# Justin900429/autonomous_driving_with_diffusion_model

Measured on AMD Instinct MI355X. Metric: denoising-steps/sec, higher is better.
Workload: dtype f32

## Files before the change

autonomous_driving_with_diffusion_model_amd/csrc/conv2d_hs.hip:

```cpp
#include <type_traits>
#include <stdlib.h>

#include "adx_common.h"
#include "conv2d_internal.h"
#include "conv2d_hs_common.h"

namespace adx {

template <bool AFFINE = true>
__device__ __forceinline__ void cells_store32(float (&v)[16], const float* sc, const float* sh, int cl0, const float (*res8)[8],
                                              bool relu, __amdgpu_buffer_rsrc_t yrsrc, uint32_t vcell, uint32_t so, uint32_t cplane,
                                              float& amax) {
  float lm = 0.f;
#pragma unroll
  for (int i = 0; i < 2; ++i)
#pragma unroll
    for (int j = 0; j < 4; ++j) {
      const auto sw = __builtin_amdgcn_permlane32_swap(f2u(v[8 * i + j]), f2u(v[8 * i + 4 + j]), false, false);
      v[8 * i + j] = u2f(sw[0]);
      v[8 * i + 4 + j] = u2f(sw[1]);
    }
#pragma unroll
  for (int i = 0; i < 2; ++i) {
    float o[8];
// ... 325 lines not shown
        if (a.relu) v = v > 0.f ? v : 0.f;
        lm = fp16_amax(lm, v);
        __builtin_amdgcn_raw_buffer_store_b32(__builtin_bit_cast(uint32_t, v), yrsrc, voff[rr], cbase_o + cu * plane_ob, 0);
        if (DS) {
          const float d = (adm[rr][half][r] + adl[rr][half][r] * (1.f / kLoScale)) * xs_inv;
          const float dv = d * ss[2 * kHsCout + cl] + ss[3 * kHsCout + cl];
          lm = fp16_amax(lm, dv);
          __builtin_amdgcn_raw_buffer_store_b32(__builtin_bit_cast(uint32_t, dv), drsrc, voff[rr], cbase_o + cu * plane_ob, 0);
        }
      }
    amax = fp16_amax(amax, voff[rr] != kOut ? lm : 0.f);
  }
  range_flag(a.status, out_of_fp16(amax));
}

#ifdef ADX_HS_TRACE
__device__ unsigned long long g_hs_trace[8 * 16384];
__device__ __forceinline__ void hs_trace(int slot) {
  if (threadIdx.x == 0 && blockIdx.x < 16384) g_hs_trace[blockIdx.x * 8 + slot] = __builtin_readcyclecounter();
}
__device__ __forceinline__ void hs_trace_id() {
  if (threadIdx.x == 0 && blockIdx.x < 16384) {
    unsigned hw, xcc;
    asm volatile("s_getreg_b32 %0, hwreg(HW_REG_HW_ID)" : "=s"(hw));
    asm volatile("s_getreg_b32 %0, hwreg(HW_REG_XCC_ID)" : "=s"(xcc));
    g_hs_trace[blockIdx.x * 8 + 7] = ((unsigned long long)xcc << 32) | hw;
  }
}
#define HS_TRACE(slot) hs_trace(slot)
#else
#define HS_TRACE(slot)
#endif

template <int MODE, int STATS = 0, bool XCELLS = false, bool YCELLS = false, bool VR = false, bool PAIR = false>
__global__ void __launch_bounds__(MODE == 0 ? 256 : 512, 2) conv2d_hs3x3_kernel(const Conv2dArgs a) {
  static_assert(!PAIR || (MODE == 0 && STATS == 0), "the PAIR form is the plain 4-wave tile");
  constexpr bool VROW = YCELLS || VR;
  constexpr int NT = MODE == 0 ? 256 : 512;
  constexpr int TH = MODE == 1 ? 16 : 8;
  constexpr int CT = MODE == 2 ? 2 : 1;
  constexpr int K = 3, PH = TH + 2, PW = 34, PLANE = PH * PW, NITEM = 2 * PLANE;
  constexpr int PIT = (NITEM + NT - 1) / NT;
  constexpr int NW = 9 * 256, WST = PAIR ? 2 * 256 : 3 * 256 * CT;
  constexpr int WIT = (WST + NT - 1) / NT;
  static_assert(PIT <= K, "a patch slice travels with each stage of a chunk");
  extern __shared__ __attribute__((aligned(16))) unsigned char smem_raw[];
  u32x4* patch = reinterpret_cast<u32x4*>(smem_raw);
  u32x4* wl = patch + 2 * 4 * PLANE;
  float* ss = reinterpret_cast<float*>(wl + 2 * WST);
  u32x4* dummy = reinterpret_cast<u32x4*>(ss + 2 * 64 * CT + 8);
  float* bsl = reinterpret_cast<float*>(dummy + 3);
  const int tid = threadIdx.x, lane = tid & 63;
  const int wave = __builtin_amdgcn_readfirstlane(tid >> 6);
  const int rowpair = MODE == 2 ? (wave & 3) : wave, slab = MODE == 2 ? (wave >> 2) : 0;
#ifdef ADX_HS_TRACE
  hs_trace_id();
#endif
  HS_TRACE(0);
  int bid = blockIdx.x;
  {
    const int per = gridDim.x >> 3;
    if (bid < per * 8) bid = (bid & 7) * per + (bid >> 3);
  }
  int kpart = 0;
  if (a.ksplit > 1) { kpart = bid % a.ksplit; bid /= a.ksplit; }
  const int ct = bid % a.cout_tiles; bid /= a.cout_tiles;
  const int tx = bid % a.tiles_x; bid /= a.tiles_x;
  const int ty = bid % a.tiles_y; bid /= a.tiles_y;
  const int n = VROW ? 0 : bid;
  const int oy0 = ty * TH, ox0 = tx * kTileW;
  const int iy0 = oy0 - a.pad, ix0 = ox0 - a.pad;
  const int cout0 = (ct * CT + slab) * kHsCout;
  const int l31 = lane & 31, khalf = lane >> 5;
  const int vx0 = tx * kTileW;
  const int ecol = PAIR ? 16 * ((lane >> 4) & 1) + (lane & 15) : l31;
  const int vl = vx0 + ecol;
  auto vdiv = [&](int v) { return (int)(((float)v + 0.5f) * a.inv_vw); };
  const int nl = VROW ? vdiv(vl) : 0, xl = VROW ? vl - nl * a.vw : 0;
  const bool lane_valid = !VROW || (nl < a.N && xl < a.W);
  const size_t hw = (size_t)a.H * a.W;
  const int nchunks_all = a.cin_pad / kHsCC;
  const int nchunks = a.ksplit > 1 ? a.cper : nchunks_all;
  const int chunk0 = kpart * nchunks;
  const float* xin = a.x + ((size_t)n * a.Cin + (size_t)chunk0 * kHsCC) * hw;
  const int nstages = nchunks * K;
  const u32x4* wsrc = reinterpret_cast<const u32x4*>(a.w) + ((size_t)ct * CT * nchunks_all + chunk0) * NW;
  constexpr uint32_t kOutside = 0xC0000000u;
  const __amdgpu_buffer_rsrc_t xrsrc = __builtin_amdgcn_make_buffer_rsrc(
      const_cast<float*>(xin), 0,
      (int)(uint32_t)((VROW ? (size_t)a.N * a.Cin : (size_t)(a.Cin - chunk0 * kHsCC)) * hw * sizeof(float)), 0x00020000);
  const uint32_t plane_bytes = (uint32_t)(hw * sizeof(float));
  uint32_t goff[PIT];
  int pcell[PIT];
#pragma unroll
  for (int k = 0; k < PIT; ++k) {
    const int e = tid + NT * k;
    const int hg = e >= PLANE ? 1 : 0;
    const int p = e - hg * PLANE;
    const int py = p / PW, px = p - py * PW;
    const int iy = iy0 + py;
    int ix = ix0 + px, ni = n;
    if constexpr (VROW) {
      const int v = vx0 - 1 + px;
      ni = vdiv(v < 0 ? 0 : v);
      ix = v - ni * a.vw;
    }
    const bool ok = e < NITEM && iy >= 0 && iy < a.H && ix >= 0 && ix < a.W && ni < a.N;
    const size_t ioff = VROW ? (size_t)ni * a.Cin * hw * sizeof(float) : 0;
    goff[k] = !ok ? kOutside
                  : XCELLS ? (uint32_t)(ioff + hg * 8 * hw * sizeof(float) + ((size_t)iy * a.W + ix) * 16)
                           : (uint32_t)(ioff + (hg * 8 * hw + (size_t)iy * a.W + ix) * sizeof(float));
    pcell[k] = e < NITEM ? hg * 2 * PLANE + p : -1;
  }
  int wsrc_off[WIT], wdst[WIT];
#pragma unroll
  for (int k = 0; k < WIT; ++k) {
    const int e = tid + NT * k;
    const int sl = e / 768, within = e - sl * 768;
    const bool ok = e < WST;
    wsrc_off[k] = ok ? sl * nchunks_all * NW + within : 0;
    wdst[k] = ok ? e : -1;
  }
  float ssv = 0.f;
  if (tid < 2 * 64 * CT) {
    const int half = tid / (64 * CT), cc = tid - half * 64 * CT;
    const int c = ct * CT * kHsCout + cc;
    ssv = a.scale == nullptr ? (half == 0 ? 1.f : 0.f) : (half == 0 ? a.scale[c] : a.shift[c]);
  }
  float bsv = 0.f;
  if (STATS == 2 && tid < 4 * 64 * CT) {
    const int which = tid / (64 * CT), cc = tid - which * 64 * CT;
    const int c = ct * CT * kHsCout + cc;
    const float mu = a.bs_mean[c], rs = a.bs_rstd[c];
    const float sc = a.bs_gamma[c] * rs;
    bsv = which == 0 ? mu : (which == 1 ? rs : (which == 2 ? sc : __builtin_fmaf(-mu, sc, a.bs_beta[c])));
  }
  float xs = 1.f, xs_inv = 1.f;
  if (a.x_amax != nullptr && a.x_amax_n < 0) {
    xs_inv = reinterpret_cast<const float*>(a.x_amax)[1];
  } else if (a.x_amax != nullptr) {
    uint32_t* red = reinterpret_cast<uint32_t*>(ss + 2 * 64 * CT);
    uint32_t b = 0;
    for (int i = tid; i < a.x_amax_n; i += NT) b = a.x_amax[i] > b ? a.x_amax[i] : b;
#pragma unroll
    for (int off = 32; off > 0; off >>= 1) {
// ... 38 lines not shown
#pragma unroll
    for (int k = 0; k < WIT; ++k) {
      u32x4* d = (WST % NT == 0 || wdst[k] >= 0) ? wl + buf * WST + wdst[k] : dummy + 2;
      *d = wv[set][k];
    }
  };
  auto load_p = [&](int chunk, int k, int set) {
    const uint32_t cbase = (uint32_t)chunk * kHsCC * plane_bytes;
    if (XCELLS) {
      const u32x4 h4 = __builtin_amdgcn_raw_buffer_load_b128(xrsrc, goff[k], cbase, 0);
      const u32x4 l4 = __builtin_amdgcn_raw_buffer_load_b128(xrsrc, goff[k], cbase + 4 * plane_bytes, 0);
#pragma unroll
      for (int j = 0; j < 4; ++j) {
        pv[set][j] = u2f(h4[j]);
        pv[set][4 + j] = u2f(l4[j]);
      }
    } else {
#pragma unroll
      for (int j = 0; j < 8; ++j)
        pv[set][j] = __builtin_bit_cast(float, __builtin_amdgcn_raw_buffer_load_b32(xrsrc, goff[k], cbase + j * plane_bytes, 0));
    }
  };
  auto store_p = [&](int set, int k, int buf) {
    u32x4 hi, lo;
    if (XCELLS) {
#pragma unroll
      for (int j = 0; j < 4; ++j) {
        hi[j] = __builtin_bit_cast(uint32_t, pv[set][j]);
        lo[j] = __builtin_bit_cast(uint32_t, pv[set][4 + j]);
      }
    } else {
      split8(pv[set], xs, hi, lo);
    }
    u32x4* pd = patch + buf * 4 * PLANE + pcell[k];
    u32x4* d0 = pcell[k] >= 0 ? pd : dummy;
    u32x4* d1 = pcell[k] >= 0 ? pd + PLANE : dummy + 1;
    *d0 = hi;
    *d1 = lo;
  };

  auto half4 = [](uint32_t h0, uint32_t h1, uint32_t l0, uint32_t l1, float* out) {
    const float inv = 1.f / kLoScale;
    asm("v_fma_mix_f32 %0, %1, %2, %3 op_sel:[0,0,0] op_sel_hi:[1,0,1]" : "=v"(out[0]) : "v"(l0), "s"(inv), "v"(h0));
    asm("v_fma_mix_f32 %0, %1, %2, %3 op_sel:[1,0,1] op_sel_hi:[1,0,1]" : "=v"(out[1]) : "v"(l0), "s"(inv), "v"(h0));
    asm("v_fma_mix_f32 %0, %1, %2, %3 op_sel:[0,0,0] op_sel_hi:[1,0,1]" : "=v"(out[2]) : "v"(l1), "s"(inv), "v"(h1));
    asm("v_fma_mix_f32 %0, %1, %2, %3 op_sel:[1,0,1] op_sel_hi:[1,0,1]" : "=v"(out[3]) : "v"(l1), "s"(inv), "v"(h1));
  };

  const int pb_lane = khalf * 2 * PLANE + (rowpair * 2) * PW + l31;
  const int wa_lane = slab * 768 + khalf * 64 + l31;

  load_w(0, 0);
  store_w(0, 0);
#pragma unroll
  for (int k = 0; k < PIT; ++k) { load_p(0, k, 0); store_p(0, k, 0); }
  load_w(1, 1);
  if (tid < 2 * 64 * CT) ss[tid] = ssv;
  if (STATS == 2 && tid < 4 * 64 * CT) bsl[tid] = bsv;
  load_p(1, 0, 1);
  HS_TRACE(1);
  __syncthreads();
  HS_TRACE(2);

  if constexpr (PAIR) {
    const int j = lane & 15, kq = lane >> 4, ts = kq >> 1, kh2 = kq & 1;
    const int npairs = nchunks >> 1;
    f32x4 am[4][4], al[4][4];
#pragma unroll
    for (int cb = 0; cb < 4; ++cb)
#pragma unroll
      for (int pb = 0; pb < 4; ++pb)
#pragma unroll
        for (int i = 0; i < 4; ++i) { am[cb][pb][i] = 0.f; al[cb][pb][i] = 0.f; }
    const u32x4* pb_g[3];
#pragma unroll
    for (int g = 0; g < 3; ++g) {
      const HsPairTap t0 = hs_pair_stage(3 * g).tap[0], t1 = hs_pair_stage(3 * g).tap[1];
      pb_g[g] = patch + kh2 * 2 * PLANE + (rowpair * 2) * PW + j + (ts ? t1.odd * 4 * PLANE + t1.kh * PW : t0.odd * 4 * PLANE + t0.kh * PW);
    }
    const int wa_pair = ts * 256 + kh2 * 64 + j;
    auto load_runs = [&](int o0, int o1, int set) {
      wv[set][0] = wsrc[o0 + tid];
      wv[set][1] = wsrc[o1 + tid];
    };
    auto pair_stages = [&](const int par, const int pair) __attribute__((always_inline)) {
      const bool more = pair + 1 < npairs;
#pragma unroll
      for (int i = 0; i < 9; ++i) {
        const int gp = (i + par) & 1;
        const HsPairStage st = hs_pair_stage(i), nx = hs_pair_stage((i + 1) % 9);
        if (i + 2 < 9) load_runs(hs_pair_run(pair, i + 2, 0), hs_pair_run(pair, i + 2, 1), gp);
        else load_runs(more ? hs_pair_run(pair + 1, i + 2 - 9, 0) : hs_pair_run(pair, 8, 0), more ? hs_pair_run(pair + 1, i + 2 - 9, 1) : hs_pair_run(pair, 8, 1), gp);
        if (nx.pround >= 0) {
          const int c = 2 * pair + 1 + (i == 8 ? 2 : nx.pnext);
          load_p(c < nchunks ? c : nchunks - 1, nx.pround, gp);
        }
        __builtin_amdgcn_sched_barrier(0);
        const u32x4* pb0 = pb_g[i / 3] + i % 3;
        const u32x4* wa0 = wl + gp * WST + wa_pair;
        f16x8 A[2][4], B[2][4];
#pragma unroll
        for (int pl = 0; pl < 2; ++pl) {
#pragma unroll
          for (int cb = 0; cb < 4; ++cb) A[pl][cb] = __builtin_bit_cast(f16x8, wa0[pl * 128 + cb * 16]);
#pragma unroll
          for (int pb = 0; pb < (XCELLS ? 4 : 2); ++pb) B[pl][pb] = __builtin_bit_cast(f16x8, pb0[pl * PLANE + (pb >> 1) * PW + (pb & 1) * 16]);
        }
#pragma unroll
        for (int pb = 0; pb < 4; ++pb) {
          if (!XCELLS && pb == 1) {
            __builtin_amdgcn_sched_barrier(0);
// ... 17 lines not shown
        __syncthreads();
      }
    };
    int pair = 0;
    for (; pair + 1 < npairs; pair += 2) {
      pair_stages(0, pair);
      pair_stages(1, pair + 1);
    }
    if (pair < npairs) pair_stages(0, pair);

    const int ox = VROW ? xl : ox0 + ecol;
    const uint32_t plane_ob = (uint32_t)(a.OH * a.OW) * (uint32_t)sizeof(float);
    const uint32_t cplane = (uint32_t)(a.OH * a.OW) * 16u;
    const size_t img = (size_t)n * a.Cout * a.OH * a.OW;
    const int img_bytes = (int)(uint32_t)((VROW ? (uint32_t)a.N : 1u) * (uint32_t)a.Cout * plane_ob);
    const uint32_t img_off = VROW ? (uint32_t)nl * (uint32_t)a.Cout * plane_ob : 0u;
    const __amdgpu_buffer_rsrc_t yrsrc = __builtin_amdgcn_make_buffer_rsrc(a.y + img, 0, img_bytes, 0x00020000);
    const __amdgpu_buffer_rsrc_t rrsrc = __builtin_amdgcn_make_buffer_rsrc(
        const_cast<float*>(a.res != nullptr ? a.res + img : a.y), 0, a.res != nullptr ? img_bytes : 0, 0x00020000);
    const uint32_t cbase_o = (uint32_t)cout0 * plane_ob;
    const uint32_t cell0 = (uint32_t)(cout0 >> 3) * 2u * cplane;
    const bool rcells = YCELLS && a.res_cells;
    bool inside[2];
    uint32_t vout[2], vres[2];
#pragma unroll
    for (int rr = 0; rr < 2; ++rr) {
      const int oy = oy0 + rowpair * 2 + rr;
      inside[rr] = lane_valid && oy < a.OH && ox < a.OW;
      const uint32_t pix = (uint32_t)(oy * a.OW + ox);
      const uint32_t vc = img_off + pix * 16u + (uint32_t)ts * 2u * cplane, vf = img_off + pix * 4u + (uint32_t)(8 * ts) * plane_ob;
      vout[rr] = !inside[rr] ? kOutside : (YCELLS ? vc : vf);
      vres[rr] = !inside[rr] ? kOutside : (rcells ? vc : vf);
    }
    uint32_t rraw[4][2][8];
#pragma unroll
    for (int cb = 0; cb < 4; ++cb)
#pragma unroll
      for (int rr = 0; rr < 2; ++rr) {
        if (rcells) {
          const uint32_t so = cell0 + (uint32_t)(2 * cb) * 2u * cplane;
          const u32x4 h4 = __builtin_amdgcn_raw_buffer_load_b128(rrsrc, vres[rr], so, 0);
          const u32x4 l4 = __builtin_amdgcn_raw_buffer_load_b128(rrsrc, vres[rr], so + cplane, 0);
#pragma unroll
          for (int c = 0; c < 4; ++c) { rraw[cb][rr][c] = h4[c]; rraw[cb][rr][4 + c] = l4[c]; }
        } else {
#pragma unroll
          for (int c = 0; c < 8; ++c)
            rraw[cb][rr][c] = __builtin_amdgcn_raw_buffer_load_b32(rrsrc, vres[rr], cbase_o + (uint32_t)(16 * cb + c) * plane_ob, 0);
        }
      }
    float amax = 0.f;
#pragma unroll
    for (int cb = 0; cb < 4; ++cb)
#pragma unroll
      for (int rr = 0; rr < 2; ++rr) {
        float o[8], r8[8];
#pragma unroll
        for (int i = 0; i < 4; ++i) {
          const int cl = 16 * cb + 4 * kq + i;
          float x = (am[cb][2 * rr][i] + al[cb][2 * rr][i] * (1.f / kLoScale)) * xs_inv;
          float y = (am[cb][2 * rr + 1][i] + al[cb][2 * rr + 1][i] * (1.f / kLoScale)) * xs_inv;
          x = x * ss[cl] + ss[64 + cl];
          y = y * ss[cl] + ss[64 + cl];
          const auto sw = __builtin_amdgcn_permlane16_swap(f2u(x), f2u(y), false, false);
          o[i] = u2f(sw[0]);
          o[4 + i] = u2f(sw[1]);
        }
        if (rcells) {
          half4(rraw[cb][rr][0], rraw[cb][rr][1], rraw[cb][rr][4], rraw[cb][rr][5], r8);
          half4(rraw[cb][rr][2], rraw[cb][rr][3], rraw[cb][rr][6], rraw[cb][rr][7], r8 + 4);
        } else {
#pragma unroll
          for (int c = 0; c < 8; ++c) r8[c] = u2f(rraw[cb][rr][c]);
        }
        float lm = 0.f;
#pragma unroll
        for (int c = 0; c < 8; ++c) {
          const float t = o[c] + r8[c];
          o[c] = a.relu ? __builtin_fmaxf(t, 0.f) : t;
          lm = fp16_amax(lm, o[c]);
        }
        amax = fp16_amax(amax, inside[rr] ? lm : 0.f);
        if constexpr (YCELLS) {
          u32x4 hi, lo;
          split8(o, 1.f, hi, lo);
          const uint32_t so = cell0 + (uint32_t)(2 * cb) * 2u * cplane;
          __builtin_amdgcn_raw_buffer_store_b128(hi, yrsrc, vout[rr], so, 0);
          __builtin_amdgcn_raw_buffer_store_b128(lo, yrsrc, vout[rr], so + cplane, 0);
          asm volatile("s_nop 0" ::"v"(hi), "v"(lo));
        } else {
#pragma unroll
          for (int c = 0; c < 8; ++c)
            __builtin_amdgcn_raw_buffer_store_b32(f2u(o[c]), yrsrc, vout[rr], cbase_o + (uint32_t)(16 * cb + c) * plane_ob, 0);
        }
      }
    range_flag(a.status, out_of_fp16(amax));
    return;
  }

  for (int cp = 0; cp < nchunks; cp += 2) {
#pragma unroll
    for (int i = 0; i < 6; ++i) {
      const int s = 3 * cp + i;
      const int kh = i % 3, cpar = (i / 3) & 1;
      const u32x4* pb0 = patch + cpar * 4 * PLANE + pb_lane;
      const u32x4* wa0 = wl + (i & 1) * WST + wa_lane;
      load_w(s + 2 < nstages ? s + 2 : nstages - 1, i & 1);
      if ((i + 1) % 3 < PIT) load_p(s + 4 < nstages ? (s + 4) / 3 : nchunks - 1, (i + 1) % 3, i & 1);
      __builtin_amdgcn_sched_barrier(0);
#pragma unroll
      for (int kw = 0; kw < K; ++kw) {
        f16x8 A[2][2], B[2][2];
#pragma unroll
        for (int pl = 0; pl < 2; ++pl) {
#pragma unroll
          for (int m = 0; m < 2; ++m) A[pl][m] = __builtin_bit_cast(f16x8, wa0[(kw * 2 + pl) * 128 + m * 32]);
#pragma unroll
          for (int r = 0; r < 2; ++r) B[pl][r] = __builtin_bit_cast(f16x8, pb0[pl * PLANE + (r + kh) * PW + kw]);
        }
#pragma unroll
        for (int r = 0; r < 2; ++r)
#pragma unroll
          for (int m = 0; m < 2; ++m) {
            accm[r][m] = hs_mfma(A[0][m], B[0][r], accm[r][m]);
            accl[r][m] = hs_mfma(A[0][m], B[1][r], accl[r][m]);
            accl[r][m] = hs_mfma(A[1][m], B[0][r], accl[r][m]);
          }
        if (kw == 0) {
          store_w((i + 1) & 1, (i + 1) & 1);
          if (i % 3 < PIT) store_p((i + 1) & 1, i % 3, ((i + 3) / 3) & 1);
        }
      }
      __syncthreads();
    }
  }

  HS_TRACE(3);
  const int ox = VROW ? xl : ox0 + ecol;
// ... 886 lines not shown

__global__ void __launch_bounds__(256) conv2d_split_reduce_kernel(const float* __restrict__ part, size_t part_stride, int nparts,
                                                                  const float* __restrict__ scale, const float* __restrict__ shift,
                                                                  const float* __restrict__ res, float* __restrict__ y,
                                                                  int cout, int plane4, size_t total4, int relu, uint32_t* status) {
  const size_t i = (size_t)blockIdx.x * 256 + threadIdx.x;
  if (i >= total4) return;
  const int c = (int)((i / plane4) % cout);
  f32x4 v = reinterpret_cast<const f32x4*>(part)[i];
  for (int p0 = 1; p0 < nparts; p0 += 8) {
    f32x4 t[8];
#pragma unroll
    for (int j = 0; j < 8; ++j) t[j] = reinterpret_cast<const f32x4*>(part + (size_t)(p0 + j < nparts ? p0 + j : 0) * part_stride)[i];
#pragma unroll
    for (int j = 0; j < 8; ++j)
      if (p0 + j < nparts) v += t[j];
  }
  const float sc = scale != nullptr ? scale[c] : 1.f, sh = shift != nullptr ? shift[c] : 0.f;
  v = v * sc + sh;
  if (res != nullptr) v += reinterpret_cast<const f32x4*>(res)[i];
  if (relu) {
#pragma unroll
    for (int k = 0; k < 4; ++k) v[k] = __builtin_fmaxf(v[k], 0.f);
  }
  reinterpret_cast<f32x4*>(y)[i] = v;
  float amax = 0.f;
#pragma unroll
  for (int k = 0; k < 4; ++k) amax = fp16_amax(amax, v[k]);
  range_flag(status, out_of_fp16(amax));
}

static constexpr size_t hs3x3_lds(int mode, int stats, bool pair = false) {
  const int th = mode == 1 ? 16 : 8, ct = mode == 2 ? 2 : 1;
  return (size_t)2 * 64 * (th + 2) * 34 + (size_t)2 * (pair ? 2 : 3 * ct) * 256 * 16 + (2 * 64 * ct + 8) * sizeof(float) + 48 +
         (stats == 2 ? 4 * 64 * ct * sizeof(float) : 0);
}
static_assert(hs3x3_lds(0, 2) <= 80 * 1024 && hs3x3_lds(1, 2) <= 160 * 1024 && hs3x3_lds(2, 2) <= 160 * 1024, "LDS budget");
static_assert(hs3x3_lds(0, 0, true) <= 80 * 1024, "LDS budget: two workgroups of the PAIR form per CU");

Hs3x3Plan conv2d_hs3x3_plan(const ConvSpec& L, const Hs3x3Query& q, const DebugSwitches& sw) {
  Hs3x3Plan p;
  p.admitted = q.fmt == 0;
  if (!hs_eligible(L, sw) || !(L.k == 3 && L.stride == 1 && L.pad == 1) || (L.cin_pad / kHsCC) % 2 != 0) return p;
  const int N = q.N, OH = q.H, OW = q.W, nchunks = L.cin_pad / kHsCC;
  int mode = L.cin < 256 ? 0 : (OH > 8 ? 1 : (L.cout % 128 == 0 ? 2 : 0));
  const long grid0 = (long)N * ceil_div(OH, 8) * ceil_div(OW, kTileW) * (L.cout / kHsCout);
  if (grid0 <= 256) mode = 0;
  if (sw.hs_mode >= 0 && !(sw.hs_mode == 2 && L.cout % 128 != 0)) mode = sw.hs_mode == 1 || sw.hs_mode == 2 ? sw.hs_mode : 0;
  const int th = mode == 1 ? 16 : 8, ct = mode == 2 ? 2 : 1;
  const bool xc = (q.fmt & kFmtXCells) != 0, yc = (q.fmt & kFmtYCells) != 0, rc = (q.fmt & kFmtResCells) != 0 && q.has_res;
  const bool xscaled = q.x_scale == kXScalePre;
  const bool in_ok = (size_t)N * L.cin * q.H * q.W * sizeof(float) < 0xC0000000u;
  const bool bytes_ok = in_ok && (size_t)N * L.cout * OH * OW * sizeof(float) < 0xC0000000u;
  const bool vfits = (long)N * (OW + 1) < (1L << 21);
  const int vw = N > 1 ? OW + 1 : OW;
  const int vtiles_x = (int)(((long)N * vw - (N > 1 ? 1 : 0) + kTileW - 1) / kTileW);
  const bool vrow_ok = sw.conv_vrow && N > 1 && vfits && bytes_ok;
  const bool q_shape = sw.hs_mode < 0 && L.cout % 128 == 0 && L.cin_pad % 64 == 0;
  const bool q_fp32out = q_shape && xc && !yc && !rc && !q.affine && vfits && bytes_ok;
  const bool q_train = q_fp32out && sw.train_cells >= 3 && !q.has_res && q.x_scale == kXScaleNone && q.bst_mask == 0;
  const bool q_dgrad = q_fp32out && sw.train_cells >= 5 && xscaled && !q.relu && (q.bst_mask == 2 || (q.bst_mask == 1 && q.bst_bits));
  const bool q_plain = q_shape && xc && yc && (!q.has_res || rc) && q.x_scale == kXScaleNone;
  const int stats_tiles = q_train || q_dgrad ? ceil_div(OH, kQTH) * vtiles_x
                                             : ceil_div(OH, th) * (!yc && !rc && vrow_ok ? vtiles_x : N * ceil_div(OW, kTileW));
  p.stats_need = (size_t)stats_tiles * (L.cout * 2 + L.cout / 64);
  const bool stats = q.stats_floats > 0 && p.stats_need <= q.stats_floats;
  const bool split_shape = mode == 0 && grid0 <= 64 && nchunks >= 8;
// ... 184 lines not shown
```

autonomous_driving_with_diffusion_model_amd/csrc/conv2d_hs16.hip:

```cpp
#include "adx_common.h"
#include "conv2d_internal.h"
#include "conv2d_hs_common.h"

namespace adx {

namespace {

typedef __attribute__((address_space(3))) void lds_void;

__device__ __forceinline__ f32x4 mfma16(f16x8 a, f16x8 b, f32x4 c) { return __builtin_amdgcn_mfma_f32_16x16x32_f16(a, b, c, 0, 0, 0); }

__device__ __forceinline__ void half4(uint32_t h0, uint32_t h1, uint32_t l0, uint32_t l1, float* out) {
  const float inv = 1.f / kLoScale;
  asm("v_fma_mix_f32 %0, %1, %2, %3 op_sel:[0,0,0] op_sel_hi:[1,0,1]" : "=v"(out[0]) : "v"(l0), "s"(inv), "v"(h0));
  asm("v_fma_mix_f32 %0, %1, %2, %3 op_sel:[1,0,1] op_sel_hi:[1,0,1]" : "=v"(out[1]) : "v"(l0), "s"(inv), "v"(h0));
  asm("v_fma_mix_f32 %0, %1, %2, %3 op_sel:[0,0,0] op_sel_hi:[1,0,1]" : "=v"(out[2]) : "v"(l1), "s"(inv), "v"(h1));
  asm("v_fma_mix_f32 %0, %1, %2, %3 op_sel:[1,0,1] op_sel_hi:[1,0,1]" : "=v"(out[3]) : "v"(l1), "s"(inv), "v"(h1));
}

}

template <bool DMA, int TRAIN = 0>
__global__ void __launch_bounds__(kQNT, 2) conv2d_hs3x3q_kernel(const Conv2dArgs a) {
  constexpr bool S2 = TRAIN == 3;
  static_assert(!S2 || DMA, "the stride-2 block entry stages with LDS-DMA only");
  constexpr int NT = kQNT, PW = kQPW, PLANE = DMA ? kQPlaneD : kQPlane, PP = DMA ? kQPlaneD : kQPlaneP, PIT = kQPit, WST = kQWst;
  constexpr int NPAIRS = DMA ? kQPairsD : kQPairs;
  constexpr int GST = DMA ? PP : 2 * PP, PLST = DMA ? 4 * PP : PP;
  extern __shared__ __attribute__((aligned(16))) unsigned char smem_raw[];
  u32x4* patch = reinterpret_cast<u32x4*>(smem_raw);
  u32x4* wl = patch + 2 * 8 * PP;
  float* ss = reinterpret_cast<float*>(wl + 2 * WST);
  u32x4* dummy = reinterpret_cast<u32x4*>(ss + 256);
  float* bsl = reinterpret_cast<float*>(dummy + 2);
  uint32_t* gnext = reinterpret_cast<uint32_t*>(bsl + 512);
  uint32_t* gpl = gnext + PIT * NT;
  const int tid = threadIdx.x, lane = tid & 63;
  const int wave = __builtin_amdgcn_readfirstlane(tid >> 6);
  const int rowpair = wave & 3, slab = wave >> 2;
  const int j = lane & 15, kq = lane >> 4;
  const int Qs = a.q_slots;
  const HsQWalk wk = hs3x3q_walk((int)(blockIdx.x & 7), (int)(blockIdx.x >> 3), a.ntiles);
  const int u_end = wk.end;
  int u = wk.first;
  if (u >= u_end) return;
  HsQUnit un = hs3x3q_unit(u, a.cout_tiles);
  int sp = un.sp, ct = un.ct;
  int ty = sp / a.tiles_x, tx = sp - ty * a.tiles_x;
  int oy0 = ty * kQTH, vx0 = tx * 32;
  auto vdiv = [&](int v) { return (int)(((float)v + 0.5f) * a.inv_vw); };
  const size_t hw = (size_t)a.H * a.W;
  const int nch16 = a.cin_pad / 16, nch32 = a.cin_pad / 32, nstages = nch32 * 9;
  constexpr uint32_t kOutside = 0xC0000000u;
  const __amdgpu_buffer_rsrc_t xrsrc = __builtin_amdgcn_make_buffer_rsrc(
      const_cast<float*>(a.x), 0, (int)(uint32_t)((size_t)a.N * a.Cin * hw * sizeof(float)), 0x00020000);
  const uint32_t plane_bytes = (uint32_t)(hw * sizeof(float));
  auto goff_of = [&](int t_, int k, int oy0_, int vx0_) -> uint32_t {
    const int e = t_ + NT * k;
    const int g = e / PLANE, p = e - g * PLANE;
    const int py = p / PW, px = p - py * PW;
// ... 104 lines not shown
    } else {
      pvh[set] = __builtin_amdgcn_raw_buffer_load_b128(xrsrc, go, cbase, 0);
      pvl[set] = __builtin_amdgcn_raw_buffer_load_b128(xrsrc, go, cbase + 4 * plane_bytes, 0);
    }
  };
  auto load_p = [&](int chunk, int k, int set) { load_p_at(chunk, k, set, goff[k]); };
  auto store_p = [&](int set, int k, int buf) {
    if constexpr (!DMA) {
      u32x4* pd = patch + buf * 8 * PP + pcell[k];
      u32x4* d0 = (k < PIT - 1 || pcell[k] >= 0) ? pd : dummy;
      u32x4* d1 = (k < PIT - 1 || pcell[k] >= 0) ? pd + PP : dummy + 1;
      *d0 = pvh[set];
      *d1 = pvl[set];
    }
  };


  if constexpr (S2) load_w_tap(ct, 0, kTap[0], 0);
  else load_w(0, 0);
  store_w(0, 0);
#pragma unroll
  for (int k = 0; k < PIT; ++k) { load_p(0, k, 0); store_p(0, k, 0); }
  if constexpr (!DMA) load_w(1, 1);
  load_consts(ct);
  if constexpr (DMA) asm volatile("s_waitcnt vmcnt(0)" ::: "memory");
  __syncthreads();

  bool bad = false;
  for (;;) {
  int zero_ = 0;
  asm volatile("" : "+s"(zero_));
  const int tl = tid + zero_;
  if constexpr (DMA && !S2) {
#pragma unroll
    for (int k = 0; k < PIT; ++k) goff[k] = goff_of(tl, k, oy0, vx0);
#pragma unroll
    for (int k = 0; k < 2; ++k) {
      const int e = tl + NT * k;
      const int sl = e >> 9, half16 = (e >> 8) & 1, within = e & 255;
      wsrc_off[k] = (((ct * 2 + sl) * nch16 + half16) * 9) * 256 + within;
    }
  }
  const int j_l = tl & 15, kq_l = (tl & 63) >> 4;
  const int pb_lane = kq_l * GST + (rowpair * 2) * PW + j_l;
  const int wa_lane = slab * 512 + (kq_l >> 1) * 256 + (kq_l & 1) * 64 + j_l;
  const int u_next = u + Qs;
  const bool has_next = DMA && u_next < u_end;
  const HsQUnit un_next = hs3x3q_unit(u_next, a.cout_tiles);
  const int sp_next = un_next.sp;
  const int ct_next = has_next ? un_next.ct : ct;
  const int wct_next = (ct_next - ct) * (2 * 9 * 256) * nch16;
  const int nty = sp_next / a.tiles_x, ntx = sp_next - nty * a.tiles_x;
  const int n_oy0 = nty * kQTH, n_vx0 = ntx * 32;
  if constexpr (S2) {
#pragma unroll
    for (int k = 0; k < PIT; ++k) {
      const uint32_t g10 = goff_s2(tl, k, oy0, vx0, 1, 0);
      gpl[(0 * PIT + k) * NT + tid] = goff_s2(tl, k, oy0, vx0, 1, 1);
      gpl[(1 * PIT + k) * NT + tid] = g10;
      gpl[(2 * PIT + k) * NT + tid] = goff_s2(tl, k, oy0, vx0, 0, 1);
      gpl[(3 * PIT + k) * NT + tid] = goff_s2(tl, k, oy0, vx0, 0, 0);
      gnext[k * NT + tid] = has_next ? goff_s2(tl, k, n_oy0, n_vx0, 1, 0) : g10;
    }
  } else if constexpr (DMA) {
#pragma unroll
    for (int k = 0; k < PIT; ++k) gnext[k * NT + tid] = has_next ? goff_of(tl, k, n_oy0, n_vx0) : goff[k];
  }
#pragma unroll
  for (int cb = 0; cb < 4; ++cb)
#pragma unroll
    for (int pb = 0; pb < 4; ++pb)
#pragma unroll
      for (int i = 0; i < 4; ++i) { accm[cb][pb][i] = 0.f; accl[cb][pb][i] = 0.f; }

  auto s2_stage = [&](const u32x4* pb0, const u32x4* wa0) {
    __builtin_amdgcn_sched_barrier(0);
    f16x8 A[2][4], B[2][4];
#pragma unroll
    for (int pl = 0; pl < 2; ++pl) {
#pragma unroll
      for (int cb = 0; cb < 4; ++cb) A[pl][cb] = __builtin_bit_cast(f16x8, wa0[pl * 128 + cb * 16]);
#pragma unroll
      for (int pb = 0; pb < 4; ++pb) B[pl][pb] = __builtin_bit_cast(f16x8, pb0[pl * PLST + (pb >> 1) * PW + (pb & 1) * 16]);
    }
#pragma unroll
    for (int pb = 0; pb < 4; ++pb) {
#pragma unroll
      for (int cb = 0; cb < 4; ++cb) {
        accm[cb][pb] = mfma16(A[0][cb], B[0][pb], accm[cb][pb]);
        accl[cb][pb] = mfma16(A[0][cb], B[1][pb], accl[cb][pb]);
// ... 262 lines not shown
            for (int k = 0; k < PIT; ++k) load_p_at(c + 1, k, (i + 1) & 1, gpl[(3 * PIT + k) * NT + tid]);
          } else {
            load_w_tap(ct_next, 0, kTap[0], 0);
#pragma unroll
            for (int k = 0; k < PIT; ++k) load_p_at(0, k, 0, gnext[k * NT + tid]);
          }
          s2_stage(patch + i * 8 * PP + pb_lane + PW + 1, wl + i * WST + wa_lane);
        }
      }
    }
  }
  float* const yout = S2 && pass == 1 ? a.y_ds : a.y;
  const float* const ssp = S2 && pass == 1 ? bsl : ss;
  const int relu = S2 && pass == 1 ? 0 : a.relu;
  const int rw = kq;
  const int vcol = vx0 + 16 * (rw & 1) + j;
  const int nl = vdiv(vcol), xl = vcol - nl * a.vw;
  const bool col_valid = nl < a.N && xl < (S2 ? a.OW : a.W);
  const uint32_t plane_ob = (uint32_t)(a.OH * a.OW) * (uint32_t)sizeof(float);
  const uint32_t cplane = (uint32_t)(a.OH * a.OW) * 16u;
  const uint32_t img_bytes = (uint32_t)a.N * (uint32_t)a.Cout * plane_ob;
  const uint32_t img_off = (uint32_t)nl * (uint32_t)a.Cout * plane_ob;
  const __amdgpu_buffer_rsrc_t yrsrc = __builtin_amdgcn_make_buffer_rsrc(yout, 0, (int)img_bytes, 0x00020000);
  const __amdgpu_buffer_rsrc_t rrsrc = __builtin_amdgcn_make_buffer_rsrc(
      const_cast<float*>(a.res != nullptr ? a.res : a.y), 0, a.res != nullptr ? (int)img_bytes : 0, 0x00020000);
  const int cout0 = ct * 128 + slab * 64;
  const uint32_t cell0 = (uint32_t)(cout0 >> 3) * 2u * cplane;
  uint32_t vcell[2];
#pragma unroll
  for (int rr = 0; rr < 2; ++rr) {
    const int oy = oy0 + rowpair * 2 + rr;
    vcell[rr] = (col_valid && oy < a.OH) ? img_off + (uint32_t)(oy * a.OW + xl) * 16u + (uint32_t)(rw >> 1) * 2u * cplane : kOutside;
  }
  u32x4 rh[4][2], rl[4][2];
#pragma unroll
  for (int cb = 0; cb < 4; ++cb)
#pragma unroll
    for (int rr = 0; rr < 2; ++rr) {
      const uint32_t so = cell0 + (uint32_t)(2 * cb) * 2u * cplane;
      if constexpr (S2) {
        rh[cb][rr] = u32x4{0u, 0u, 0u, 0u};
        rl[cb][rr] = u32x4{0u, 0u, 0u, 0u};
      } else {
        rh[cb][rr] = __builtin_amdgcn_raw_buffer_load_b128(rrsrc, vcell[rr], so, 0);
        rl[cb][rr] = __builtin_amdgcn_raw_buffer_load_b128(rrsrc, vcell[rr], so + cplane, 0);
      }
    }
  const float* sc = ssp + slab * 64;
  const float* sh = ssp + 128 + slab * 64;
  float am[2] = {0.f, 0.f};
#pragma unroll
  for (int cb = 0; cb < 4; ++cb)
#pragma unroll
    for (int rr = 0; rr < 2; ++rr) {
      float x[4], y[4];
#pragma unroll
      for (int i = 0; i < 4; ++i) {
        const int cl = cb * 16 + 4 * kq + i;
        x[i] = (accm[cb][2 * rr][i] + accl[cb][2 * rr][i] * (1.f / kLoScale)) * sc[cl] + sh[cl];
        y[i] = (accm[cb][2 * rr + 1][i] + accl[cb][2 * rr + 1][i] * (1.f / kLoScale)) * sc[cl] + sh[cl];
      }
      float o[8];
#pragma unroll
      for (int i = 0; i < 4; ++i) {
        const auto sw = __builtin_amdgcn_permlane16_swap(f2u(x[i]), f2u(y[i]), false, false);
        o[i] = u2f(sw[0]);
        o[4 + i] = u2f(sw[1]);
      }
      float r8[8];
      half4(rh[cb][rr][0], rh[cb][rr][1], rl[cb][rr][0], rl[cb][rr][1], r8);
      half4(rh[cb][rr][2], rh[cb][rr][3], rl[cb][rr][2], rl[cb][rr][3], r8 + 4);
#pragma unroll
      for (int i = 0; i < 8; ++i) {
        const float tsum = o[i] + r8[i];
        o[i] = relu ? __builtin_fmaxf(tsum, 0.f) : tsum;
        am[rr] = fp16_amax(am[rr], o[i]);
      }
      u32x4 hi, lo;
      split8(o, 1.f, hi, lo);
      const uint32_t so = cell0 + (uint32_t)(2 * cb) * 2u * cplane;
      __builtin_amdgcn_raw_buffer_store_b128(hi, yrsrc, vcell[rr], so, 0);
      __builtin_amdgcn_raw_buffer_store_b128(lo, yrsrc, vcell[rr], so + cplane, 0);
      asm volatile("s_nop 0" ::"v"(hi), "v"(lo));
    }
  bad |= ((vcell[0] != kOutside) & out_of_fp16(am[0])) | ((vcell[1] != kOutside) & out_of_fp16(am[1]));
  } while (S2 && ++pass < 2);
  }
  if (!has_next) break;
  if constexpr (TRAIN == 1 || TRAIN == 2) __syncthreads();
  if (ct_next != ct) {
    if constexpr (TRAIN == 0 || S2) __syncthreads();
    load_consts(ct_next);
  }
  u += Qs;
  asm volatile("" : "+s"(u));
  un = hs3x3q_unit(u, a.cout_tiles);
  sp = un.sp; ct = un.ct;
  ty = sp / a.tiles_x; tx = sp - ty * a.tiles_x;
  oy0 = ty * kQTH; vx0 = tx * 32;
  }
  range_flag(a.status, bad);
}

int conv2d_hs3x3q_launch(const Hs3x3Plan& p, Conv2dArgs a, hipStream_t s) {
  typedef void (*QKernel)(const Conv2dArgs);
  static const QKernel table[2][3] = {
      {&conv2d_hs3x3q_kernel<false, 0>, &conv2d_hs3x3q_kernel<false, 1>, &conv2d_hs3x3q_kernel<false, 2>},
      {&conv2d_hs3x3q_kernel<true, 0>, &conv2d_hs3x3q_kernel<true, 1>, &conv2d_hs3x3q_kernel<true, 2>}};
  static std::atomic<uint64_t> attr{0};
  if (DeviceOnce once{attr}; once) {
    for (int dma = 0; dma < 2; ++dma)
      for (const QKernel k : table[dma])
        ADX_CHECK_HIP(hipFuncSetAttribute(reinterpret_cast<const void*>(k), hipFuncAttributeMaxDynamicSharedMemorySize, (int)(dma ? kQLdsD : kQLds)));
    once.commit();
  }
  ADX_REQUIRE((long)a.N * p.vw < (1L << 21), "conv2d_hs: batch x width exceeds the virtual-row arithmetic");
  const size_t tiles = (size_t)p.cout_tiles * p.tiles_x * p.tiles_y;
  ADX_REQUIRE(tiles < (1u << 31), "conv2d_hs: grid too large");
  ADX_REQUIRE((size_t)a.N * a.Cout * a.OH * a.OW * sizeof(float) < 0xC0000000u && (size_t)a.N * a.Cin * a.H * a.W * sizeof(float) < 0xC0000000u,
              "conv2d_hs: a cell-layout tensor exceeds the 32-bit byte offsets");
  a.vw = p.vw; a.inv_vw = 1.f / (float)p.vw;
  a.tiles_x = p.tiles_x; a.tiles_y = p.tiles_y; a.cout_tiles = p.cout_tiles; a.ntiles = (int)tiles;
  a.q_slots = p.q_slots;
  a.ksplit = p.ksplit; a.cper = p.cper; a.part = nullptr;
  table[p.dma][p.stats]<<<dim3((unsigned)p.grid), dim3(p.threads), p.lds, s>>>(a);
  ADX_LAUNCH_CHECK();
  return ADX_OK;
}

int conv2d_hs3x3q_s2_launch(const HsS2Plan& p, Conv2dArgs a, hipStream_t s) {
  static std::atomic<uint64_t> attr{0};
  if (DeviceOnce once{attr}; once) {
// ... 16 lines not shown
```

Measured before the change: 172.6.

## Pad PAIR patch k-half pitch, specialize residual/relu epilogues, reuse precomputed offsets

The PAIR form of the 3x3 conv kernel now places each k-half of the LDS patch at a padded pitch of 688 cells, so the half-patches start on whole bank rounds. This is meant to cut LDS bank conflicts, at the cost of a slightly larger LDS footprint. The residual epilogues in both kernels are specialized at compile time, so the residual loads are skipped when no residual tensor exists. The hs16 epilogue also fixes relu as a constant and computes the scale/shift FMAs as two-wide vectors to allow packed math. In the DMA inference path, the next tile's gather offsets are read from a precomputed LDS table instead of being recomputed, and the gnext table is assumed to be filled elsewhere.

```diff
diff --git a/autonomous_driving_with_diffusion_model_amd/csrc/conv2d_hs.hip b/autonomous_driving_with_diffusion_model_amd/csrc/conv2d_hs.hip
--- a/autonomous_driving_with_diffusion_model_amd/csrc/conv2d_hs.hip
+++ b/autonomous_driving_with_diffusion_model_amd/csrc/conv2d_hs.hip
@@ -381,6 +381,8 @@
 #define HS_TRACE(slot)
 #endif
 
+constexpr int kHsPairKHalf = 688;
+static_assert(kHsPairKHalf % 16 == 0 && kHsPairKHalf >= 2 * 10 * 34, "the k-half pitch of the PAIR form: whole bank rounds, two planes");
 template <int MODE, int STATS = 0, bool XCELLS = false, bool YCELLS = false, bool VR = false, bool PAIR = false>
 __global__ void __launch_bounds__(MODE == 0 ? 256 : 512, 2) conv2d_hs3x3_kernel(const Conv2dArgs a) {
   static_assert(!PAIR || (MODE == 0 && STATS == 0), "the PAIR form is the plain 4-wave tile");
@@ -389,13 +391,15 @@
   constexpr int TH = MODE == 1 ? 16 : 8;
   constexpr int CT = MODE == 2 ? 2 : 1;
   constexpr int K = 3, PH = TH + 2, PW = 34, PLANE = PH * PW, NITEM = 2 * PLANE;
+  constexpr int KHP = PAIR ? kHsPairKHalf : 2 * PLANE, COPY = 2 * KHP;
+  static_assert(KHP >= 2 * PLANE, "a k-half holds its two planes");
   constexpr int PIT = (NITEM + NT - 1) / NT;
   constexpr int NW = 9 * 256, WST = PAIR ? 2 * 256 : 3 * 256 * CT;
   constexpr int WIT = (WST + NT - 1) / NT;
   static_assert(PIT <= K, "a patch slice travels with each stage of a chunk");
   extern __shared__ __attribute__((aligned(16))) unsigned char smem_raw[];
   u32x4* patch = reinterpret_cast<u32x4*>(smem_raw);
-  u32x4* wl = patch + 2 * 4 * PLANE;
+  u32x4* wl = patch + 2 * COPY;
   float* ss = reinterpret_cast<float*>(wl + 2 * WST);
   u32x4* dummy = reinterpret_cast<u32x4*>(ss + 2 * 64 * CT + 8);
   float* bsl = reinterpret_cast<float*>(dummy + 3);
@@ -459,7 +463,7 @@
     goff[k] = !ok ? kOutside
                   : XCELLS ? (uint32_t)(ioff + hg * 8 * hw * sizeof(float) + ((size_t)iy * a.W + ix) * 16)
                            : (uint32_t)(ioff + (hg * 8 * hw + (size_t)iy * a.W + ix) * sizeof(float));
-    pcell[k] = e < NITEM ? hg * 2 * PLANE + p : -1;
+    pcell[k] = e < NITEM ? hg * KHP + p : -1;
   }
   int wsrc_off[WIT], wdst[WIT];
 #pragma unroll
@@ -564,7 +568,7 @@
     } else {
       split8(pv[set], xs, hi, lo);
     }
-    u32x4* pd = patch + buf * 4 * PLANE + pcell[k];
+    u32x4* pd = patch + buf * COPY + pcell[k];
     u32x4* d0 = pcell[k] >= 0 ? pd : dummy;
     u32x4* d1 = pcell[k] >= 0 ? pd + PLANE : dummy + 1;
     *d0 = hi;
@@ -579,7 +583,7 @@
     asm("v_fma_mix_f32 %0, %1, %2, %3 op_sel:[1,0,1] op_sel_hi:[1,0,1]" : "=v"(out[3]) : "v"(l1), "s"(inv), "v"(h1));
   };
 
-  const int pb_lane = khalf * 2 * PLANE + (rowpair * 2) * PW + l31;
+  const int pb_lane = khalf * KHP + (rowpair * 2) * PW + l31;
   const int wa_lane = slab * 768 + khalf * 64 + l31;
 
   load_w(0, 0);
@@ -608,7 +612,7 @@
 #pragma unroll
     for (int g = 0; g < 3; ++g) {
       const HsPairTap t0 = hs_pair_stage(3 * g).tap[0], t1 = hs_pair_stage(3 * g).tap[1];
-      pb_g[g] = patch + kh2 * 2 * PLANE + (rowpair * 2) * PW + j + (ts ? t1.odd * 4 * PLANE + t1.kh * PW : t0.odd * 4 * PLANE + t0.kh * PW);
+      pb_g[g] = patch + kh2 * KHP + (rowpair * 2) * PW + j + (ts ? t1.odd * COPY + t1.kh * PW : t0.odd * COPY + t0.kh * PW);
     }
     const int wa_pair = ts * 256 + kh2 * 64 + j;
     auto load_runs = [&](int o0, int o1, int set) {
@@ -692,68 +696,78 @@
       vout[rr] = !inside[rr] ? kOutside : (YCELLS ? vc : vf);
       vres[rr] = !inside[rr] ? kOutside : (rcells ? vc : vf);
     }
-    uint32_t rraw[4][2][8];
-#pragma unroll
-    for (int cb = 0; cb < 4; ++cb)
-#pragma unroll
-      for (int rr = 0; rr < 2; ++rr) {
-        if (rcells) {
-          const uint32_t so = cell0 + (uint32_t)(2 * cb) * 2u * cplane;
-          const u32x4 h4 = __builtin_amdgcn_raw_buffer_load_b128(rrsrc, vres[rr], so, 0);
-          const u32x4 l4 = __builtin_amdgcn_raw_buffer_load_b128(rrsrc, vres[rr], so + cplane, 0);
-#pragma unroll
-          for (int c = 0; c < 4; ++c) { rraw[cb][rr][c] = h4[c]; rraw[cb][rr][4 + c] = l4[c]; }
-        } else {
-#pragma unroll
-          for (int c = 0; c < 8; ++c)
-            rraw[cb][rr][c] = __builtin_amdgcn_raw_buffer_load_b32(rrsrc, vres[rr], cbase_o + (uint32_t)(16 * cb + c) * plane_ob, 0);
-        }
-      }
     float amax = 0.f;
-#pragma unroll
-    for (int cb = 0; cb < 4; ++cb)
-#pragma unroll
-      for (int rr = 0; rr < 2; ++rr) {
-        float o[8], r8[8];
-#pragma unroll
-        for (int i = 0; i < 4; ++i) {
-          const int cl = 16 * cb + 4 * kq + i;
-          float x = (am[cb][2 * rr][i] + al[cb][2 * rr][i] * (1.f / kLoScale)) * xs_inv;
-          float y = (am[cb][2 * rr + 1][i] + al[cb][2 * rr + 1][i] * (1.f / kLoScale)) * xs_inv;
-          x = x * ss[cl] + ss[64 + cl];
-          y = y * ss[cl] + ss[64 + cl];
-          const auto sw = __builtin_amdgcn_permlane16_swap(f2u(x), f2u(y), false, false);
-          o[i] = u2f(sw[0]);
-          o[4 + i] = u2f(sw[1]);
-        }
-        if (rcells) {
-          half4(rraw[cb][rr][0], rraw[cb][rr][1], rraw[cb][rr][4], rraw[cb][rr][5], r8);
-          half4(rraw[cb][rr][2], rraw[cb][rr][3], rraw[cb][rr][6], rraw[cb][rr][7], r8 + 4);
-        } else {
-#pragma unroll
-          for (int c = 0; c < 8; ++c) r8[c] = u2f(rraw[cb][rr][c]);
-        }
-        float lm = 0.f;
-#pragma unroll
-        for (int c = 0; c < 8; ++c) {
-          const float t = o[c] + r8[c];
-          o[c] = a.relu ? __builtin_fmaxf(t, 0.f) : t;
-          lm = fp16_amax(lm, o[c]);
-        }
-        amax = fp16_amax(amax, inside[rr] ? lm : 0.f);
-        if constexpr (YCELLS) {
-          u32x4 hi, lo;
-          split8(o, 1.f, hi, lo);
-          const uint32_t so = cell0 + (uint32_t)(2 * cb) * 2u * cplane;
-          __builtin_amdgcn_raw_buffer_store_b128(hi, yrsrc, vout[rr], so, 0);
-          __builtin_amdgcn_raw_buffer_store_b128(lo, yrsrc, vout[rr], so + cplane, 0);
-          asm volatile("s_nop 0" ::"v"(hi), "v"(lo));
-        } else {
-#pragma unroll
-          for (int c = 0; c < 8; ++c)
-            __builtin_amdgcn_raw_buffer_store_b32(f2u(o[c]), yrsrc, vout[rr], cbase_o + (uint32_t)(16 * cb + c) * plane_ob, 0);
-        }
-      }
+    auto finish = [&](auto res_c) __attribute__((always_inline)) {
+      constexpr bool RES = decltype(res_c)::value;
+      uint32_t rraw[4][2][8];
+      if constexpr (RES) {
+#pragma unroll
+        for (int cb = 0; cb < 4; ++cb)
+#pragma unroll
+          for (int rr = 0; rr < 2; ++rr) {
+            if (rcells) {
+              const uint32_t so = cell0 + (uint32_t)(2 * cb) * 2u * cplane;
+              const u32x4 h4 = __builtin_amdgcn_raw_buffer_load_b128(rrsrc, vres[rr], so, 0);
+              const u32x4 l4 = __builtin_amdgcn_raw_buffer_load_b128(rrsrc, vres[rr], so + cplane, 0);
+#pragma unroll
+              for (int c = 0; c < 4; ++c) { rraw[cb][rr][c] = h4[c]; rraw[cb][rr][4 + c] = l4[c]; }
+            } else {
+#pragma unroll
+              for (int c = 0; c < 8; ++c)
+                rraw[cb][rr][c] = __builtin_amdgcn_raw_buffer_load_b32(rrsrc, vres[rr], cbase_o + (uint32_t)(16 * cb + c) * plane_ob, 0);
+            }
+          }
+      }
+#pragma unroll
+      for (int cb = 0; cb < 4; ++cb)
+#pragma unroll
+        for (int rr = 0; rr < 2; ++rr) {
+          float o[8], r8[8];
+#pragma unroll
+          for (int i = 0; i < 4; ++i) {
+            const int cl = 16 * cb + 4 * kq + i;
+            float x = (am[cb][2 * rr][i] + al[cb][2 * rr][i] * (1.f / kLoScale)) * xs_inv;
+            float y = (am[cb][2 * rr + 1][i] + al[cb][2 * rr + 1][i] * (1.f / kLoScale)) * xs_inv;
+            x = x * ss[cl] + ss[64 + cl];
+            y = y * ss[cl] + ss[64 + cl];
+            const auto sw = __builtin_amdgcn_permlane16_swap(f2u(x), f2u(y), false, false);
+            o[i] = u2f(sw[0]);
+            o[4 + i] = u2f(sw[1]);
+          }
+          if constexpr (!RES) {
+#pragma unroll
+            for (int c = 0; c < 8; ++c) r8[c] = 0.f;
+          } else if (rcells) {
+            half4(rraw[cb][rr][0], rraw[cb][rr][1], rraw[cb][rr][4], rraw[cb][rr][5], r8);
+            half4(rraw[cb][rr][2], rraw[cb][rr][3], rraw[cb][rr][6], rraw[cb][rr][7], r8 + 4);
+          } else {
+#pragma unroll
+            for (int c = 0; c < 8; ++c) r8[c] = u2f(rraw[cb][rr][c]);
+          }
+          float lm = 0.f;
+#pragma unroll
+          for (int c = 0; c < 8; ++c) {
+            const float t = o[c] + r8[c];
+            o[c] = a.relu ? __builtin_fmaxf(t, 0.f) : t;
+            lm = fp16_amax(lm, o[c]);
+          }
+          amax = fp16_amax(amax, inside[rr] ? lm : 0.f);
+          if constexpr (YCELLS) {
+            u32x4 hi, lo;
+            split8(o, 1.f, hi, lo);
+            const uint32_t so = cell0 + (uint32_t)(2 * cb) * 2u * cplane;
+            __builtin_amdgcn_raw_buffer_store_b128(hi, yrsrc, vout[rr], so, 0);
+            __builtin_amdgcn_raw_buffer_store_b128(lo, yrsrc, vout[rr], so + cplane, 0);
+            asm volatile("s_nop 0" ::"v"(hi), "v"(lo));
+          } else {
+#pragma unroll
+            for (int c = 0; c < 8; ++c)
+              __builtin_amdgcn_raw_buffer_store_b32(f2u(o[c]), yrsrc, vout[rr], cbase_o + (uint32_t)(16 * cb + c) * plane_ob, 0);
+          }
+        }
+    };
+    if (!XCELLS || a.res != nullptr) finish(std::true_type{});
+    else finish(std::false_type{});
     range_flag(a.status, out_of_fp16(amax));
     return;
   }
@@ -763,7 +777,7 @@
     for (int i = 0; i < 6; ++i) {
       const int s = 3 * cp + i;
       const int kh = i % 3, cpar = (i / 3) & 1;
-      const u32x4* pb0 = patch + cpar * 4 * PLANE + pb_lane;
+      const u32x4* pb0 = patch + cpar * COPY + pb_lane;
       const u32x4* wa0 = wl + (i & 1) * WST + wa_lane;
       load_w(s + 2 < nstages ? s + 2 : nstages - 1, i & 1);
       if ((i + 1) % 3 < PIT) load_p(s + 4 < nstages ? (s + 4) / 3 : nchunks - 1, (i + 1) % 3, i & 1);
@@ -1716,7 +1730,8 @@
 
 static constexpr size_t hs3x3_lds(int mode, int stats, bool pair = false) {
   const int th = mode == 1 ? 16 : 8, ct = mode == 2 ? 2 : 1;
-  return (size_t)2 * 64 * (th + 2) * 34 + (size_t)2 * (pair ? 2 : 3 * ct) * 256 * 16 + (2 * 64 * ct + 8) * sizeof(float) + 48 +
+  const size_t patch = pair ?(size_t)2 * 2 * kHsPairKHalf * 16 : (size_t)2 * 64 * (th + 2) * 34;
+  return patch + (size_t)2 * (pair ? 2 : 3 * ct) * 256 * 16 + (2 * 64 * ct + 8) * sizeof(float) + 48 +
          (stats == 2 ? 4 * 64 * ct * sizeof(float) : 0);
 }
 static_assert(hs3x3_lds(0, 2) <= 80 * 1024 && hs3x3_lds(1, 2) <= 160 * 1024 && hs3x3_lds(2, 2) <= 160 * 1024, "LDS budget");
diff --git a/autonomous_driving_with_diffusion_model_amd/csrc/conv2d_hs16.hip b/autonomous_driving_with_diffusion_model_amd/csrc/conv2d_hs16.hip
--- a/autonomous_driving_with_diffusion_model_amd/csrc/conv2d_hs16.hip
+++ b/autonomous_driving_with_diffusion_model_amd/csrc/conv2d_hs16.hip
@@ -7,6 +7,7 @@
 namespace {
 
 typedef __attribute__((address_space(3))) void lds_void;
+typedef float f32x2 __attribute__((ext_vector_type(2)));
 
 __device__ __forceinline__ f32x4 mfma16(f16x8 a, f16x8 b, f32x4 c) { return __builtin_amdgcn_mfma_f32_16x16x32_f16(a, b, c, 0, 0, 0); }
 
@@ -26,6 +27,7 @@
   static_assert(!S2 || DMA, "the stride-2 block entry stages with LDS-DMA only");
   constexpr int NT = kQNT, PW = kQPW, PLANE = DMA ? kQPlaneD : kQPlane, PP = DMA ? kQPlaneD : kQPlaneP, PIT = kQPit, WST = kQWst;
   constexpr int NPAIRS = DMA ? kQPairsD : kQPairs;
+  constexpr bool HAND = DMA && (TRAIN == 0 || S2);
   constexpr int GST = DMA ? PP : 2 * PP, PLST = DMA ? 4 * PP : PP;
   extern __shared__ __attribute__((aligned(16))) unsigned char smem_raw[];
   u32x4* patch = reinterpret_cast<u32x4*>(smem_raw);
@@ -196,8 +198,10 @@
   asm volatile("" : "+s"(zero_));
   const int tl = tid + zero_;
   if constexpr (DMA && !S2) {
-#pragma unroll
-    for (int k = 0; k < PIT; ++k) goff[k] = goff_of(tl, k, oy0, vx0);
+    if constexpr (!HAND) {
+#pragma unroll
+      for (int k = 0; k < PIT; ++k) goff[k] = goff_of(tl, k, oy0, vx0);
+    }
 #pragma unroll
     for (int k = 0; k < 2; ++k) {
       const int e = tl + NT * k;
@@ -219,7 +223,7 @@
   if constexpr (S2) {
 #pragma unroll
     for (int k = 0; k < PIT; ++k) {
-      const uint32_t g10 = goff_s2(tl, k, oy0, vx0, 1, 0);
+      const uint32_t g10 = HAND ? goff[k] : goff_s2(tl, k, oy0, vx0, 1, 0);
       gpl[(0 * PIT + k) * NT + tid] = goff_s2(tl, k, oy0, vx0, 1, 1);
       gpl[(1 * PIT + k) * NT + tid] = g10;
       gpl[(2 * PIT + k) * NT + tid] = goff_s2(tl, k, oy0, vx0, 0, 1);
@@ -548,57 +552,79 @@
     const int oy = oy0 + rowpair * 2 + rr;
     vcell[rr] = (col_valid && oy < a.OH) ? img_off + (uint32_t)(oy * a.OW + xl) * 16u + (uint32_t)(rw >> 1) * 2u * cplane : kOutside;
   }
-  u32x4 rh[4][2], rl[4][2];
-#pragma unroll
-  for (int cb = 0; cb < 4; ++cb)
-#pragma unroll
-    for (int rr = 0; rr < 2; ++rr) {
-      const uint32_t so = cell0 + (uint32_t)(2 * cb) * 2u * cplane;
-      if constexpr (S2) {
-        rh[cb][rr] = u32x4{0u, 0u, 0u, 0u};
-        rl[cb][rr] = u32x4{0u, 0u, 0u, 0u};
-      } else {
-        rh[cb][rr] = __builtin_amdgcn_raw_buffer_load_b128(rrsrc, vcell[rr], so, 0);
-        rl[cb][rr] = __builtin_amdgcn_raw_buffer_load_b128(rrsrc, vcell[rr], so + cplane, 0);
-      }
-    }
   const float* sc = ssp + slab * 64;
   const float* sh = ssp + 128 + slab * 64;
   float am[2] = {0.f, 0.f};
-#pragma unroll
-  for (int cb = 0; cb < 4; ++cb)
-#pragma unroll
-    for (int rr = 0; rr < 2; ++rr) {
-      float x[4], y[4];
-#pragma unroll
-      for (int i = 0; i < 4; ++i) {
-        const int cl = cb * 16 + 4 * kq + i;
-        x[i] = (accm[cb][2 * rr][i] + accl[cb][2 * rr][i] * (1.f / kLoScale)) * sc[cl] + sh[cl];
-        y[i] = (accm[cb][2 * rr + 1][i] + accl[cb][2 * rr + 1][i] * (1.f / kLoScale)) * sc[cl] + sh[cl];
-      }
-      float o[8];
-#pragma unroll
-      for (int i = 0; i < 4; ++i) {
-        const auto sw = __builtin_amdgcn_permlane16_swap(f2u(x[i]), f2u(y[i]), false, false);
-        o[i] = u2f(sw[0]);
-        o[4 + i] = u2f(sw[1]);
-      }
-      float r8[8];
-      half4(rh[cb][rr][0], rh[cb][rr][1], rl[cb][rr][0], rl[cb][rr][1], r8);
-      half4(rh[cb][rr][2], rh[cb][rr][3], rl[cb][rr][2], rl[cb][rr][3], r8 + 4);
-#pragma unroll
-      for (int i = 0; i < 8; ++i) {
-        const float tsum = o[i] + r8[i];
-        o[i] = relu ? __builtin_fmaxf(tsum, 0.f) : tsum;
-        am[rr] = fp16_amax(am[rr], o[i]);
-      }
-      u32x4 hi, lo;
-      split8(o, 1.f, hi, lo);
-      const uint32_t so = cell0 + (uint32_t)(2 * cb) * 2u * cplane;
-      __builtin_amdgcn_raw_buffer_store_b128(hi, yrsrc, vcell[rr], so, 0);
-      __builtin_amdgcn_raw_buffer_store_b128(lo, yrsrc, vcell[rr], so + cplane, 0);
-      asm volatile("s_nop 0" ::"v"(hi), "v"(lo));
-    }
+  auto cells_out = [&](auto res_c, auto relu_c) __attribute__((always_inline)) {
+    constexpr bool RES = decltype(res_c)::value, RELU = decltype(relu_c)::value;
+    u32x4 rh[4][2], rl[4][2];
+    if constexpr (RES) {
+#pragma unroll
+      for (int cb = 0; cb < 4; ++cb)
+#pragma unroll
+        for (int rr = 0; rr < 2; ++rr) {
+          const uint32_t so = cell0 + (uint32_t)(2 * cb) * 2u * cplane;
+          rh[cb][rr] = __builtin_amdgcn_raw_buffer_load_b128(rrsrc, vcell[rr], so, 0);
+          rl[cb][rr] = __builtin_amdgcn_raw_buffer_load_b128(rrsrc, vcell[rr], so + cplane, 0);
+        }
+    }
+#pragma unroll
+    for (int cb = 0; cb < 4; ++cb)
+#pragma unroll
+      for (int rr = 0; rr < 2; ++rr) {
+        float x[4], y[4];
+#pragma unroll
+        for (int h = 0; h < 2; ++h) {
+          const int cl = cb * 16 + 4 * kq + 2 * h;
+          const f32x2 inv2 = {1.f / kLoScale, 1.f / kLoScale};
+          const f32x2 sc2 = {sc[cl], sc[cl + 1]}, sh2 = {sh[cl], sh[cl + 1]};
+          const f32x2 xm = {accm[cb][2 * rr][2 * h], accm[cb][2 * rr][2 * h + 1]}, xl2 = {accl[cb][2 * rr][2 * h], accl[cb][2 * rr][2 * h + 1]};
+          const f32x2 ym = {accm[cb][2 * rr + 1][2 * h], accm[cb][2 * rr + 1][2 * h + 1]};
+          const f32x2 yl2 = {accl[cb][2 * rr + 1][2 * h], accl[cb][2 * rr + 1][2 * h + 1]};
+          const f32x2 xv = __builtin_elementwise_fma(__builtin_elementwise_fma(xl2, inv2, xm), sc2, sh2);
+          const f32x2 yv = __builtin_elementwise_fma(__builtin_elementwise_fma(yl2, inv2, ym), sc2, sh2);
+          x[2 * h] = xv[0]; x[2 * h + 1] = xv[1];
+          y[2 * h] = yv[0]; y[2 * h + 1] = yv[1];
+        }
+        float o[8];
+#pragma unroll
+        for (int i = 0; i < 4; ++i) {
+          const auto sw = __builtin_amdgcn_permlane16_swap(f2u(x[i]), f2u(y[i]), false, false);
+          o[i] = u2f(sw[0]);
+          o[4 + i] = u2f(sw[1]);
+        }
+        float r8[8];
+        if constexpr (RES) {
+          half4(rh[cb][rr][0], rh[cb][rr][1], rl[cb][rr][0], rl[cb][rr][1], r8);
+          half4(rh[cb][rr][2], rh[cb][rr][3], rl[cb][rr][2], rl[cb][rr][3], r8 + 4);
+        } else {
+#pragma unroll
+          for (int i = 0; i < 8; ++i) r8[i] = 0.f;
+        }
+#pragma unroll
+        for (int i = 0; i < 8; ++i) {
+          const float tsum = o[i] + r8[i];
+          o[i] = RELU ? __builtin_fmaxf(tsum, 0.f) : tsum;
+          am[rr] = fp16_amax(am[rr], o[i]);
+        }
+        u32x4 hi, lo;
+        split8(o, 1.f, hi, lo);
+        const uint32_t so = cell0 + (uint32_t)(2 * cb) * 2u * cplane;
+        __builtin_amdgcn_raw_buffer_store_b128(hi, yrsrc, vcell[rr], so, 0);
+        __builtin_amdgcn_raw_buffer_store_b128(lo, yrsrc, vcell[rr], so + cplane, 0);
+        asm volatile("s_nop 0" ::"v"(hi), "v"(lo));
+      }
+  };
+  using std::false_type;
+  using std::true_type;
+  const bool with_res = !S2 && a.res != nullptr;
+  if (relu) {
+    if (with_res) cells_out(true_type{}, true_type{});
+    else cells_out(false_type{}, true_type{});
+  } else {
+    if (with_res) cells_out(true_type{}, false_type{});
+    else cells_out(false_type{}, false_type{});
+  }
   bad |= ((vcell[0] != kOutside) & out_of_fp16(am[0])) | ((vcell[1] != kOutside) & out_of_fp16(am[1]));
   } while (S2 && ++pass < 2);
   }
@@ -614,6 +640,10 @@
   sp = un.sp; ct = un.ct;
   ty = sp / a.tiles_x; tx = sp - ty * a.tiles_x;
   oy0 = ty * kQTH; vx0 = tx * 32;
+  if constexpr (HAND) {
+#pragma unroll
+    for (int k = 0; k < PIT; ++k) goff[k] = gnext[k * NT + tid];
+  }
   }
   range_flag(a.status, bad);
 }
```

New measurement: 174.6, median of 6. +1.1%, better.
